# sun-huangqingbo/multiplexed-image-annotator

Measured on AMD Instinct MI355X. Metric: cells/sec annotated (whole node), higher is better.
Workload: dtype f16

## Files before the change

multiplexed-image-annotator_amd/csrc/cell_attention.hip:

```cpp

#include "gemm_epi.h"
#include "ribca_common.h"
#include "ribca_kernels.h"

namespace ribca {

namespace {

typedef __attribute__((__vector_size__(4 * sizeof(_Float16)))) _Float16 f16x4c;
typedef __attribute__((__vector_size__(4 * sizeof(short)))) short s16x4c;
__device__ __forceinline__ f16x4c lds_read_tr16c(const char* p) {
  return __builtin_bit_cast(f16x4c, __builtin_amdgcn_ds_read_tr16_b64_v4i16((s16x4c __attribute__((address_space(3)))*)(p)));
}

constexpr int kTP = 112, kVRows = 128;

template <int D, int HD> struct CellGeom {
  static constexpr int Dp = (D + 31) / 32 * 32;
  static constexpr int NK = Dp / 32;
  static constexpr int GD = HD == 32 ? 64 : 48;
  static constexpr int NTP = GD / 16;
  static constexpr int WROWS = 3 * GD;
  static constexpr int WSTAGE = WROWS * ROWB;
  static constexpr int GROUPS = D / GD;
  static constexpr int HPG = GD / HD;
  static constexpr int KIMG = kTP * ROWB;
  static constexpr int VROWB = 4 * GD;
  static constexpr int VIMG = kVRows * VROWB + 64;
  static constexpr int CB = 2 * 3 * D * 4;
  static constexpr int RING = 3;
  static constexpr int OFF_K = RING * WSTAGE;
  static constexpr int OFF_V = OFF_K + HPG * KIMG;
  static constexpr int OFF_CB = OFF_V + (VIMG + 15) / 16 * 16;
  static constexpr int LDS = OFF_CB + CB;
  static_assert(D % GD == 0 && GD % HD == 0 && HD % 4 == 0 && HD <= 32 && HPG % 2 == 0 && WROWS % 8 == 0, "head geometry");
};

}

template <int D, int HD>
__global__ __launch_bounds__(512) void cell_qkv_attention_kernel(const uint16_t* __restrict__ z, int ldz, const uint16_t* __restrict__ W, int ldw,
                                                                 const float* __restrict__ bias2, const float* __restrict__ csum,
                                                                 const float2* __restrict__ rowstat, uint16_t* __restrict__ out, int ldo, int T,
                                                                 float scale) {
  using G = CellGeom<D, HD>;
  constexpr int NK = G::NK, GROUPS = G::GROUPS, HPG = G::HPG, kRing = G::RING, kGroupDims = G::GD, NTP = G::NTP, kWStage = G::WSTAGE;
  constexpr int NTILES = 3 * NTP;
  constexpr int TOTAL = GROUPS * NK;
  constexpr int GPL = G::WROWS / 8;
  extern __shared__ __attribute__((aligned(16))) char smem[];
  const int tid = threadIdx.x, lane = tid & 63;
  const int wave = __builtin_amdgcn_readfirstlane(tid >> 6);
  const int cell = blockIdx.x;
  const int r16 = lane & 15, g = lane >> 4;

  for (int i = tid; i < 3 * D / 4; i += 512) {
    reinterpret_cast<float4*>(smem + G::OFF_CB)[i] = reinterpret_cast<const float4*>(csum)[i];
    reinterpret_cast<float4*>(smem + G::OFF_CB + 3 * D * 4)[i] = reinterpret_cast<const float4*>(bias2)[i];
  }
  for (int o = kTP * G::VROWB + tid * 16; o < G::VIMG; o += 512 * 16) *reinterpret_cast<uint4*>(smem + G::OFF_V + o) = uint4{0u, 0u, 0u, 0u};
  __syncthreads();

  if (wave == 7) {
    auto issue = [&](int step) {
      const int hg = step / NK, s = step - hg * NK;
      char* st = smem + (step % kRing) * kWStage;
#pragma unroll
      for (int i = 0; i < GPL; ++i) {
        const int row = i * 8 + (lane >> 3);
        const int which = row / kGroupDims, c = row - which * kGroupDims;
        const int n = which * D + hg * kGroupDims + c;
        const int ch = (lane & 7) ^ swz_f(row);
        const uint16_t* src = W + (size_t)n * ldw + s * (2 * BK) + ch * 8;
        __builtin_amdgcn_global_load_lds((const __attribute__((address_space(1))) void*)src, (__attribute__((address_space(3))) void*)(st + i * 1024), 16,
                                         0, 0);
      }
    };
    issue(0);
    issue(1);
    for (int step = 0; step < TOTAL; ++step) {
      if (step + 1 < TOTAL) wait_vmcnt<GPL>();
      else wait_vmcnt<0>();
      __builtin_amdgcn_s_barrier();
      asm volatile("" ::: "memory");
      if (step + 2 < TOTAL) issue(step + 2);
      if ((step + 1) % NK == 0) __builtin_amdgcn_s_barrier();
    }
    return;
  }

  const int tok = wave * 16 + r16;
  const int trow = tok < T ? tok : T - 1;
  const uint16_t* zr = z + ((size_t)cell * T + trow) * ldz;
  f16x8 ahi[NK], alo[NK];
#pragma unroll
  for (int s = 0; s < NK; ++s) {
    const uint4* p = reinterpret_cast<const uint4*>(zr + (4 * s + g) * 16);
    ahi[s] = __builtin_bit_cast(f16x8, p[0]);
    alo[s] = __builtin_bit_cast(f16x8, p[1]);
  }
  const float2 rs = rowstat[(size_t)cell * T + trow];
  const float rstd = rs.x, nm = -rs.y * rs.x;
  const char* cb = smem + G::OFF_CB;
  uint16_t* orow = out + ((size_t)cell * T + tok) * ldo;
  int w_rd[NTILES];
#pragma unroll
  for (int j = 0; j < NTILES; ++j) w_rd[j] = lds_off(16 * j + r16, 2 * g);
  const int k_wr = lds_off(tok, 2 * g);
  constexpr int KST = 4, NT = 7;

  int step = 0;
  for (int hg = 0; hg < GROUPS; ++hg) {
    f32x4 acc[NTILES];
#pragma unroll
    for (int j = 0; j < NTILES; ++j) acc[j] = f32x4{0.f, 0.f, 0.f, 0.f};
#pragma unroll
    for (int s = 0; s < NK; ++s, ++step) {
      asm volatile("s_waitcnt lgkmcnt(0)" ::: "memory");
      __builtin_amdgcn_s_barrier();
      asm volatile("" ::: "memory");
      const char* st = smem + (step % kRing) * kWStage;
#pragma unroll
      for (int jb = 0; jb < NTILES / 3; ++jb) {
        f16x8 whi[3], wlo[3];
#pragma unroll
        for (int j = 0; j < 3; ++j) {
          whi[j] = __builtin_bit_cast(f16x8, *reinterpret_cast<const uint4*>(st + w_rd[3 * jb + j]));
          wlo[j] = __builtin_bit_cast(f16x8, *reinterpret_cast<const uint4*>(st + (w_rd[3 * jb + j] ^ 16)));
        }
#pragma unroll
        for (int j = 0; j < 3; ++j) acc[3 * jb + j] = mfma_f16(wlo[j], ahi[s], acc[3 * jb + j]);
#pragma unroll
        for (int j = 0; j < 3; ++j) acc[3 * jb + j] = mfma_f16(whi[j], alo[s], acc[3 * jb + j]);
#pragma unroll
        for (int j = 0; j < 3; ++j) acc[3 * jb + j] = mfma_f16(whi[j], ahi[s], acc[3 * jb + j]);
      }
    }
#pragma unroll
    for (int j = 0; j < NTILES; ++j) {
      const int n = (j / NTP) * D + hg * kGroupDims + 16 * (j % NTP) + 4 * g;
      const float4 c4 = *reinterpret_cast<const float4*>(cb + n * 4), b4 = *reinterpret_cast<const float4*>(cb + 3 * D * 4 + n * 4);
      const f32x2v r2 = {rstd, rstd}, n2 = {nm, nm};
      const f32x2v lo2 = fma2(r2, f32x2v{acc[j][0], acc[j][1]}, fma2(n2, f32x2v{c4.x, c4.y}, f32x2v{b4.x, b4.y}));
      const f32x2v hi2 = fma2(r2, f32x2v{acc[j][2], acc[j][3]}, fma2(n2, f32x2v{c4.z, c4.w}, f32x2v{b4.z, b4.w}));
      acc[j] = f32x4{lo2.x, lo2.y, hi2.x, hi2.y};
    }
    f16x8 qhi[HPG], qlo[HPG];
#pragma unroll
    for (int h = 0; h < HPG; ++h) {
      constexpr int dummy = 0; (void)dummy;
      const int d_lo = h * HD, d_hi = d_lo + HD;
      const int tA = d_lo / 16, tB = (d_hi - 1) / 16;
      const bool inA = 16 * tA + 4 * g >= d_lo && 16 * tA + 4 * g < d_hi;
      const bool inB = tB != tA && 16 * tB + 4 * g >= d_lo && 16 * tB + 4 * g < d_hi;
      float qa[4], qb[4], ka[4], kb[4];
#pragma unroll
      for (int r = 0; r < 4; ++r) {
        qa[r] = inA ? acc[tA][r] * scale : 0.f;
        qb[r] = inB ? acc[tB][r] * scale : 0.f;
        ka[r] = inA ? acc[NTP + tA][r] : 0.f;
        kb[r] = inB ? acc[NTP + tB][r] : 0.f;
      }
      uint2 h0, l0, h1, l1;
      split4(qa, h0, l0);
      split4(qb, h1, l1);
      qhi[h] = __builtin_bit_cast(f16x8, uint4{h0.x, h0.y, h1.x, h1.y});
      qlo[h] = __builtin_bit_cast(f16x8, uint4{l0.x, l0.y, l1.x, l1.y});
      split4(ka, h0, l0);
      split4(kb, h1, l1);
      char* kimg = smem + G::OFF_K + h * G::KIMG;
      *reinterpret_cast<uint4*>(kimg + k_wr) = uint4{h0.x, h0.y, h1.x, h1.y};
      *reinterpret_cast<uint4*>(kimg + (k_wr ^ 16)) = uint4{l0.x, l0.y, l1.x, l1.y};
    }
    {
      uint16_t* vrow = reinterpret_cast<uint16_t*>(smem + G::OFF_V + tok * G::VROWB);
#pragma unroll
      for (int j = 0; j < NTP; ++j) {
        const float v4[4] = {acc[2 * NTP + j][0], acc[2 * NTP + j][1], acc[2 * NTP + j][2], acc[2 * NTP + j][3]};
        const int jj = kGroupDims == 64 ? (j ^ (tok & 3)) : j;
        ps_store4_pair<16>(vrow, 16 * jj + 4 * g, v4);
      }
    }
    asm volatile("s_waitcnt lgkmcnt(0)" ::: "memory");
    __builtin_amdgcn_s_barrier();
    asm volatile("" ::: "memory");

    constexpr int DT = (HD + 15) / 16;
    const char* vimg = smem + G::OFF_V;
#pragma unroll
    for (int hp = 0; hp < HPG; hp += 2) {
      f32x4 s[2][2 * KST];
#pragma unroll
      for (int kt = 0; kt < NT; ++kt) {
        const int ko = lds_off(16 * kt + r16, 2 * g);
#pragma unroll
        for (int e = 0; e < 2; ++e) {
          const char* kimg = smem + G::OFF_K + (hp + e) * G::KIMG;
          const f16x8 kh = __builtin_bit_cast(f16x8, *reinterpret_cast<const uint4*>(kimg + ko));
          const f16x8 kl = __builtin_bit_cast(f16x8, *reinterpret_cast<const uint4*>(kimg + (ko ^ 16)));
          s[e][kt] = f32x4{0.f, 0.f, 0.f, 0.f};
          s[e][kt] = mfma_f16(kl, qhi[hp + e], s[e][kt]);
          s[e][kt] = mfma_f16(kh, qlo[hp + e], s[e][kt]);
          s[e][kt] = mfma_f16(kh, qhi[hp + e], s[e][kt]);
        }
      }
      f16x8 phi[2][KST], plo[2][KST];
#pragma unroll
      for (int e = 0; e < 2; ++e) {
#pragma unroll
        for (int r = 0; r < 4; ++r)
          if (16 * (NT - 1) + 4 * g + r >= T) s[e][NT - 1][r] = -INFINITY;
        float mx = -INFINITY;
#pragma unroll
        for (int kt = 0; kt < NT; ++kt)
#pragma unroll
          for (int r = 0; r < 4; ++r) mx = fmaxf(mx, s[e][kt][r]);
        mx = fmaxf(mx, __shfl_xor(mx, 16, 64));
        mx = fmaxf(mx, __shfl_xor(mx, 32, 64));
        const f32x2v l2 = {1.44269504089f, 1.44269504089f}, moff = {-mx * 1.44269504089f, -mx * 1.44269504089f};
        f32x2v sum2 = {0.f, 0.f};
#pragma unroll
        for (int kt = 0; kt < NT; ++kt) {
          const f32x2v a0 = fma2(f32x2v{s[e][kt][0], s[e][kt][1]}, l2, moff);
          const f32x2v a1 = fma2(f32x2v{s[e][kt][2], s[e][kt][3]}, l2, moff);
          const f32x2v e0 = {__builtin_amdgcn_exp2f(a0.x), __builtin_amdgcn_exp2f(a0.y)}, e1 = {__builtin_amdgcn_exp2f(a1.x), __builtin_amdgcn_exp2f(a1.y)};
          s[e][kt] = f32x4{e0.x, e0.y, e1.x, e1.y};
          sum2 += e0;
          sum2 += e1;
        }
        float sum = sum2.x + sum2.y;
        sum += __shfl_xor(sum, 16, 64);
        sum += __shfl_xor(sum, 32, 64);
        const float inv = 1.0f / sum;
        const f32x2v inv2 = {inv, inv};
        s[e][NT] = f32x4{0.f, 0.f, 0.f, 0.f};
#pragma unroll
        for (int t = 0; t < KST; ++t) {
          const f32x2v pa0 = f32x2v{s[e][2 * t][0], s[e][2 * t][1]} * inv2, pa1 = f32x2v{s[e][2 * t][2], s[e][2 * t][3]} * inv2;
          const f32x2v pb0 = f32x2v{s[e][2 * t + 1][0], s[e][2 * t + 1][1]} * inv2, pb1 = f32x2v{s[e][2 * t + 1][2], s[e][2 * t + 1][3]} * inv2;
          const float pa[4] = {pa0.x, pa0.y, pa1.x, pa1.y}, pb[4] = {pb0.x, pb0.y, pb1.x, pb1.y};
          uint2 ha, la, hb, lb;
          split4_unit(pa, ha, la);
          split4_unit(pb, hb, lb);
          phi[e][t] = __builtin_bit_cast(f16x8, uint4{ha.x, ha.y, hb.x, hb.y});
          plo[e][t] = __builtin_bit_cast(f16x8, uint4{la.x, la.y, lb.x, lb.y});
        }
      }
#pragma unroll
      for (int dt = 0; dt < DT; ++dt) {
        f32x4 o[2] = {f32x4{0.f, 0.f, 0.f, 0.f}, f32x4{0.f, 0.f, 0.f, 0.f}};
#pragma unroll
        for (int t = 0; t < KST; ++t) {
#pragma unroll
          for (int e = 0; e < 2; ++e) {
            const int dcol0 = (hp + e) * HD + 16 * dt + 4 * (r16 & 3);
            const int dcol = kGroupDims == 64 ? ((((dcol0 >> 4) ^ (r16 >> 2)) << 4) | (dcol0 & 15)) : dcol0;
            const int voff = (dcol >> 3) * 32 + (dcol & 7) * 2;
            const char* va = vimg + (32 * t + 4 * g + (r16 >> 2)) * G::VROWB + voff;
            const f16x4c h0 = lds_read_tr16c(va), l0 = lds_read_tr16c(va + 16);
            const f16x4c h1 = lds_read_tr16c(va + 16 * G::VROWB), l1 = lds_read_tr16c(va + 16 * G::VROWB + 16);
            const f16x8 vhi = __builtin_shufflevector(h0, h1, 0, 1, 2, 3, 4, 5, 6, 7);
            const f16x8 vlo = __builtin_shufflevector(l0, l1, 0, 1, 2, 3, 4, 5, 6, 7);
            o[e] = mfma_f16(vlo, phi[e][t], o[e]);
            o[e] = mfma_f16(vhi, plo[e][t], o[e]);
            o[e] = mfma_f16(vhi, phi[e][t], o[e]);
          }
        }
        const int d = 16 * dt + 4 * g;
        if (tok < T && d < HD) {
#pragma unroll
          for (int e = 0; e < 2; ++e) {
            const float v4[4] = {o[e][0], o[e][1], o[e][2], o[e][3]};
            ps_store4(orow, (hg * HPG + hp + e) * HD + d, v4);
          }
        }
      }
    }
  }
}

bool cell_attention_supported(int D, int H, int T) { return H == kHeads && T == kTokens && (D == 144 || D == 288 || D == 384); }

void launch_cell_qkv_attention(const uint16_t* z, int ldz, const uint16_t* W, int ldw, const float* bias2, const float* csum, const float2* rowstat,
                               uint16_t* out, int ldo, int cells, int D, float scale, hipStream_t s) {
  if (cells <= 0) return;
  auto go = [&](auto kern, int lds) {
    static unsigned long long attr_done[3] = {0ull, 0ull, 0ull};
    const int slot = D == 288 ? 1 : D == 384 ? 2 : 0;
    if (!ensure_dynamic_lds(reinterpret_cast<const void*>(kern), lds, attr_done[slot])) return;
    hipLaunchKernelGGL(kern, dim3(cells), dim3(512), lds, s, z, ldz, W, ldw, bias2, csum, rowstat, out, ldo, (int)kTokens, scale);
  };
  if (D == 288) go(cell_qkv_attention_kernel<288, 24>, CellGeom<288, 24>::LDS);
  else if (D == 384) go(cell_qkv_attention_kernel<384, 32>, CellGeom<384, 32>::LDS);
  else go(cell_qkv_attention_kernel<144, 12>, CellGeom<144, 12>::LDS);
}

}
```

Measured before the change: 17270.

## Software-pipeline K/V LDS reads in cell attention and use permlane swaps for reductions

For D=384, K-tile and V-tile LDS reads are issued a fixed number of steps ahead of the MFMAs that use them, and sched_barrier pins keep the compiler from reordering this schedule. For the other D values, the cross-lane max and sum reductions use permlane16/32 swap instructions in place of shuffle-xor. W-tile read addresses are now computed from a base offset plus a constant stride instead of a per-tile array. The lookahead raises register pressure and the pinned schedule may limit the compiler's own interleaving.

```diff
diff --git a/multiplexed-image-annotator_amd/csrc/cell_attention.hip b/multiplexed-image-annotator_amd/csrc/cell_attention.hip
--- a/multiplexed-image-annotator_amd/csrc/cell_attention.hip
+++ b/multiplexed-image-annotator_amd/csrc/cell_attention.hip
@@ -12,6 +12,30 @@
 __device__ __forceinline__ f16x4c lds_read_tr16c(const char* p) {
   return __builtin_bit_cast(f16x4c, __builtin_amdgcn_ds_read_tr16_b64_v4i16((s16x4c __attribute__((address_space(3)))*)(p)));
 }
+
+template <bool kLaneSwap, typename Op>
+__device__ __forceinline__ float xor16_32(float v, Op op) {
+  if constexpr (!kLaneSwap) {
+    v = op(v, __shfl_xor(v, 16, 64));
+    return op(v, __shfl_xor(v, 32, 64));
+  }
+  const uint32_t u = __builtin_bit_cast(uint32_t, v);
+  const auto a = __builtin_amdgcn_permlane16_swap(u, u, false, false);
+  const uint32_t a0 = a[0], a1 = a[1];
+  const uint32_t w = __builtin_bit_cast(uint32_t, op(__builtin_bit_cast(float, a0), __builtin_bit_cast(float, a1)));
+  const auto b = __builtin_amdgcn_permlane32_swap(w, w, false, false);
+  const uint32_t b0 = b[0], b1 = b[1];
+  return op(__builtin_bit_cast(float, b0), __builtin_bit_cast(float, b1));
+}
+
+template <bool kPin> __device__ __forceinline__ void pin() {
+  if constexpr (kPin) __builtin_amdgcn_sched_barrier(0);
+}
+
+template <int D> struct CellAhead {
+  static constexpr int K = D == 384 ? 2 : 0, V = D == 384 ? 1 : 0;
+  static constexpr bool kLaneSwap = D != 384;
+};
 
 constexpr int kTP = 112, kVRows = 128;
 
@@ -103,9 +127,7 @@
   const float rstd = rs.x, nm = -rs.y * rs.x;
   const char* cb = smem + G::OFF_CB;
   uint16_t* orow = out + ((size_t)cell * T + tok) * ldo;
-  int w_rd[NTILES];
-#pragma unroll
-  for (int j = 0; j < NTILES; ++j) w_rd[j] = lds_off(16 * j + r16, 2 * g);
+  const int f_hi = lds_off(r16, 2 * g), f_lo = f_hi ^ 16;
   const int k_wr = lds_off(tok, 2 * g);
   constexpr int KST = 4, NT = 7;
 
@@ -124,10 +146,9 @@
       for (int jb = 0; jb < NTILES / 3; ++jb) {
         f16x8 whi[3], wlo[3];
 #pragma unroll
-        for (int j = 0; j < 3; ++j) {
-          whi[j] = __builtin_bit_cast(f16x8, *reinterpret_cast<const uint4*>(st + w_rd[3 * jb + j]));
-          wlo[j] = __builtin_bit_cast(f16x8, *reinterpret_cast<const uint4*>(st + (w_rd[3 * jb + j] ^ 16)));
-        }
+        for (int j = 0; j < 3; ++j) wlo[j] = __builtin_bit_cast(f16x8, *reinterpret_cast<const uint4*>(st + f_lo + (3 * jb + j) * 16 * ROWB));
+#pragma unroll
+        for (int j = 0; j < 3; ++j) whi[j] = __builtin_bit_cast(f16x8, *reinterpret_cast<const uint4*>(st + f_hi + (3 * jb + j) * 16 * ROWB));
 #pragma unroll
         for (int j = 0; j < 3; ++j) acc[3 * jb + j] = mfma_f16(wlo[j], ahi[s], acc[3 * jb + j]);
 #pragma unroll
@@ -190,19 +211,35 @@
 #pragma unroll
     for (int hp = 0; hp < HPG; hp += 2) {
       f32x4 s[2][2 * KST];
+      constexpr int kKAhead = CellAhead<D>::K;
+      f16x8 kh[NT][2], kl[NT][2];
+      auto read_k = [&](int kt) {
+#pragma unroll
+        for (int e = 0; e < 2; ++e) {
+          const char* kimg = smem + G::OFF_K + (hp + e) * G::KIMG + kt * 16 * ROWB;
+          kl[kt][e] = __builtin_bit_cast(f16x8, *reinterpret_cast<const uint4*>(kimg + f_lo));
+          pin<(kKAhead > 0)>();
+          kh[kt][e] = __builtin_bit_cast(f16x8, *reinterpret_cast<const uint4*>(kimg + f_hi));
+          pin<(kKAhead > 0)>();
+        }
+      };
+#pragma unroll
+      for (int kt = 0; kt < kKAhead; ++kt) read_k(kt);
+      pin<(kKAhead > 0)>();
 #pragma unroll
       for (int kt = 0; kt < NT; ++kt) {
-        const int ko = lds_off(16 * kt + r16, 2 * g);
+        if (kt + kKAhead < NT) {
+          read_k(kt + kKAhead);
+          pin<(kKAhead > 0)>();
+        }
 #pragma unroll
         for (int e = 0; e < 2; ++e) {
-          const char* kimg = smem + G::OFF_K + (hp + e) * G::KIMG;
-          const f16x8 kh = __builtin_bit_cast(f16x8, *reinterpret_cast<const uint4*>(kimg + ko));
-          const f16x8 kl = __builtin_bit_cast(f16x8, *reinterpret_cast<const uint4*>(kimg + (ko ^ 16)));
           s[e][kt] = f32x4{0.f, 0.f, 0.f, 0.f};
-          s[e][kt] = mfma_f16(kl, qhi[hp + e], s[e][kt]);
-          s[e][kt] = mfma_f16(kh, qlo[hp + e], s[e][kt]);
-          s[e][kt] = mfma_f16(kh, qhi[hp + e], s[e][kt]);
-        }
+          s[e][kt] = mfma_f16(kl[kt][e], qhi[hp + e], s[e][kt]);
+          s[e][kt] = mfma_f16(kh[kt][e], qlo[hp + e], s[e][kt]);
+          s[e][kt] = mfma_f16(kh[kt][e], qhi[hp + e], s[e][kt]);
+        }
+        if (kt + 1 < NT) pin<(kKAhead > 0)>();
       }
       f16x8 phi[2][KST], plo[2][KST];
 #pragma unroll
@@ -215,8 +252,7 @@
         for (int kt = 0; kt < NT; ++kt)
 #pragma unroll
           for (int r = 0; r < 4; ++r) mx = fmaxf(mx, s[e][kt][r]);
-        mx = fmaxf(mx, __shfl_xor(mx, 16, 64));
-        mx = fmaxf(mx, __shfl_xor(mx, 32, 64));
+        mx = xor16_32<CellAhead<D>::kLaneSwap>(mx, [](float a, float b) { return fmaxf(a, b); });
         const f32x2v l2 = {1.44269504089f, 1.44269504089f}, moff = {-mx * 1.44269504089f, -mx * 1.44269504089f};
         f32x2v sum2 = {0.f, 0.f};
 #pragma unroll
@@ -229,8 +265,7 @@
           sum2 += e1;
         }
         float sum = sum2.x + sum2.y;
-        sum += __shfl_xor(sum, 16, 64);
-        sum += __shfl_xor(sum, 32, 64);
+        sum = xor16_32<CellAhead<D>::kLaneSwap>(sum, [](float a, float b) { return a + b; });
         const float inv = 1.0f / sum;
         const f32x2v inv2 = {inv, inv};
         s[e][NT] = f32x4{0.f, 0.f, 0.f, 0.f};
@@ -246,25 +281,42 @@
           plo[e][t] = __builtin_bit_cast(f16x8, uint4{la.x, la.y, lb.x, lb.y});
         }
       }
+      constexpr int kVAhead = CellAhead<D>::V, kVSteps = DT * KST;
+      f16x8 vhi[kVSteps][2], vlo[kVSteps][2];
+      auto read_v = [&](int u) {
+        const int dt = u / KST, t = u - dt * KST;
+#pragma unroll
+        for (int e = 0; e < 2; ++e) {
+          const int dcol0 = (hp + e) * HD + 16 * dt + 4 * (r16 & 3);
+          const int dcol = kGroupDims == 64 ? ((((dcol0 >> 4) ^ (r16 >> 2)) << 4) | (dcol0 & 15)) : dcol0;
+          const int voff = (dcol >> 3) * 32 + (dcol & 7) * 2;
+          const char* va = vimg + (32 * t + 4 * g + (r16 >> 2)) * G::VROWB + voff;
+          const f16x4c h0 = lds_read_tr16c(va), l0 = lds_read_tr16c(va + 16);
+          const f16x4c h1 = lds_read_tr16c(va + 16 * G::VROWB), l1 = lds_read_tr16c(va + 16 * G::VROWB + 16);
+          vhi[u][e] = __builtin_shufflevector(h0, h1, 0, 1, 2, 3, 4, 5, 6, 7);
+          vlo[u][e] = __builtin_shufflevector(l0, l1, 0, 1, 2, 3, 4, 5, 6, 7);
+        }
+      };
+#pragma unroll
+      for (int u = 0; u < kVAhead; ++u) read_v(u);
+      pin<(kVAhead > 0)>();
 #pragma unroll
       for (int dt = 0; dt < DT; ++dt) {
         f32x4 o[2] = {f32x4{0.f, 0.f, 0.f, 0.f}, f32x4{0.f, 0.f, 0.f, 0.f}};
 #pragma unroll
         for (int t = 0; t < KST; ++t) {
+          const int u = dt * KST + t;
+          if (u + kVAhead < kVSteps) {
+            read_v(u + kVAhead);
+            pin<(kVAhead > 0)>();
+          }
 #pragma unroll
           for (int e = 0; e < 2; ++e) {
-            const int dcol0 = (hp + e) * HD + 16 * dt + 4 * (r16 & 3);
-            const int dcol = kGroupDims == 64 ? ((((dcol0 >> 4) ^ (r16 >> 2)) << 4) | (dcol0 & 15)) : dcol0;
-            const int voff = (dcol >> 3) * 32 + (dcol & 7) * 2;
-            const char* va = vimg + (32 * t + 4 * g + (r16 >> 2)) * G::VROWB + voff;
-            const f16x4c h0 = lds_read_tr16c(va), l0 = lds_read_tr16c(va + 16);
-            const f16x4c h1 = lds_read_tr16c(va + 16 * G::VROWB), l1 = lds_read_tr16c(va + 16 * G::VROWB + 16);
-            const f16x8 vhi = __builtin_shufflevector(h0, h1, 0, 1, 2, 3, 4, 5, 6, 7);
-            const f16x8 vlo = __builtin_shufflevector(l0, l1, 0, 1, 2, 3, 4, 5, 6, 7);
-            o[e] = mfma_f16(vlo, phi[e][t], o[e]);
-            o[e] = mfma_f16(vhi, plo[e][t], o[e]);
-            o[e] = mfma_f16(vhi, phi[e][t], o[e]);
+            o[e] = mfma_f16(vlo[u][e], phi[e][t], o[e]);
+            o[e] = mfma_f16(vhi[u][e], plo[e][t], o[e]);
+            o[e] = mfma_f16(vhi[u][e], phi[e][t], o[e]);
           }
+          pin<(kVAhead > 0)>();
         }
         const int d = 16 * dt + 4 * g;
         if (tok < T && d < HD) {
```

Measured after the change: 17320 (median of 3 runs). No clear change (+0.3%).
